# NingZhang1/pyscf_isdf

Measured on AMD Instinct MI355X. Metric: isdf_build_plus_get_jk_wall_time, lower is better.
Workload: dtype f64

## Files before the change

### include/mi355_isdf.h

```cpp
#ifndef MI355_ISDF_H
#define MI355_ISDF_H

#include <stdint.h>

#ifdef __cplusplus
extern "C" {
#endif

typedef struct isdf_ctx* isdf_handle;

#define ISDF_OK 0
#define ISDF_ERR_ARG 1
#define ISDF_ERR_HIP 2
#define ISDF_ERR_LIB 3
#define ISDF_ERR_NUM 4

int isdf_abi_version(void);

int isdf_create(int device_id, isdf_handle* out);
int isdf_destroy(isdf_handle h);
int isdf_set_stream(isdf_handle h, void* hip_stream);
const char* isdf_last_error(isdf_handle h);
int64_t isdf_workspace_bytes(isdf_handle h);
int isdf_release_workspace(isdf_handle h);
// ... 82 lines not shown
                    const int64_t* d_ip, int P, double reg_rel, double* d_theta, int64_t ldt,
                    double* d_aoP, double* reg_used);

int isdf_gather_aoP(isdf_handle h, const double* d_ao, int nao, int64_t ld, const int64_t* d_ip, int P,
                    double* d_aoP);
int isdf_gram_sq(isdf_handle h, const double* d_aoP, int P, int nao, int nh, double* d_A);
int isdf_pair_gram_rows(isdf_handle h, const double* d_aoP, int P, int nao, int nh, const double* d_ao,
                        int64_t ng, int64_t ld, double* d_B, int64_t ldb);
int isdf_block_chol(isdf_handle h, const double* d_A, int P, int nblk, const int32_t* blk_off,
                    double shift_rel, double* d_D, double* shift_used);
int isdf_block_solve(isdf_handle h, const double* d_D, int P, int nblk, const int32_t* blk_off, int side,
                     int trans, double* d_X, int64_t n, int64_t ldx);
int isdf_block_invert(isdf_handle h, const double* d_D, int P, int nblk, const int32_t* blk_off, double* d_Dinv);
int isdf_block_apply(isdf_handle h, const double* d_Dinv, int64_t ldd, int nblk, const int32_t* blk_off,
                     double* d_X, int64_t n, int64_t ldx);
int isdf_pair_rows_block_apply(isdf_handle h, const double* d_aoP, int P, int nao, const double* d_ao, int64_t ng,
                               int64_t ld, const double* d_Dinv, int64_t ldd, int nblk, const int32_t* blk_off,
                               double* d_B, int64_t ldb);
int isdf_pair_rows_squared(isdf_handle h, const double* d_aoP, int rows, int nao, const double* d_ao, int64_t ng,
                           int64_t ld, int* squared);
int isdf_pair_rows_frontier(isdf_handle h, const double* d_aoP, int nnew, int nao, const double* d_ao, int64_t ng,
                            int64_t ld, int squared, const double* d_Dinv, int64_t ldd, int nblk, const int32_t* blk_off,
                            double* d_B, int64_t ldb, int have);

int isdf_gram_prod(isdf_handle h, const double* d_aoP, int P, int nao, const double* d_psiP, int nocc, double* d_A);
int isdf_pair_prod_rows(isdf_handle h, const double* d_aoP, int P, int nao, const double* d_psiP, int nocc,
                        const double* d_ao, int64_t ld, const double* d_psi, int64_t ldpsi, int64_t ng,
                        double* d_B, int64_t ldb);
int isdf_factor_solve_half(isdf_handle h, const double* d_fac, int P, int backward, double* d_X, int64_t n, int64_t ldx);
int isdf_gram_prod_cplx(isdf_handle h, const double* d_aoP, int P, int nao, int nh, const double* d_psiP, int npsi, int npsi_h,
                        double* d_A);
int isdf_pair_prod_rows_cplx(isdf_handle h, const double* d_aoP, int P, int nao, int nh, const double* d_psiP, int npsi,
                             int npsi_h, const double* d_ao, int64_t ld, const double* d_psi, int64_t ldpsi, int64_t ng,
                             double* d_B, int64_t ldb);

int isdf_shift_diag(isdf_handle h, double* d_A, int P, double shift_rel);
int isdf_chol_inplace(isdf_handle h, double* d_A, int P, double shift_rel, double* d_scratch, double* reg_used);

int isdf_factor_solve(isdf_handle h, const double* d_fac, int P, double* d_X, int64_t n, int64_t ldx);

int isdf_bj_probe_vectors(isdf_handle h, double* d_T, int n, const double* d_fac, const double* d_D, int P,
                          int nblk, const int32_t* blk_off);
int isdf_rows_combine(isdf_handle h, const double* d_E, int n, int64_t ldE, int rows, const double* d_Y,
                      int64_t ng, int64_t ldy, double* d_F, int64_t ldf, int accumulate);

int isdf_bj_probe_rows(isdf_handle h, double* d_T, int n, const double* d_fac, const double* d_D, int P, int nblk,
// ... 136 lines not shown
```

### pyscf_isdf_amd/backend.py

```python
import ctypes
import os
import numpy as np
import torch
from . import lib as _lib

_vp = ctypes.c_void_p


def _np_ptr(a):
    return a.ctypes.data_as(_vp)


class HipBackend:
    name = 'hip-gfx950'

    def __init__(self, device=0):
        if not torch.cuda.is_available():
            raise _lib.IsdfError('no GPU visible to torch; the ISDF path has no CPU fallback')
        self.device = torch.device('cuda', device)
        torch.cuda.set_device(self.device)
        self.handle = _lib.Handle(device)
        if os.environ.get('ISDF_TRSM') == 'subst':
            self.set_option('trsm_substitution', 1)
        if os.environ.get('ISDF_OWN_FFT') in ('0', '1', '2'):
# ... 286 lines not shown
        self._stream()
        blk_off = np.ascontiguousarray(blk_off, dtype=np.int32)
        assert aoP.stride(1) == 1 and aoP.stride(0) == aoP.shape[1]
        self.handle.call('isdf_pair_rows_block_apply', self._p(aoP), aoP.shape[0], aoP.shape[1], self._p(ao), int(ng), ao.stride(0),
                         self._p(Dinv), Dinv.stride(0), len(blk_off) - 1, _np_ptr(blk_off), self._p(B), B.stride(0))

    def pair_rows_squared(self, aoP, rows, ao, ng):
        self._stream()
        sq = ctypes.c_int(0)
        self.handle.call('isdf_pair_rows_squared', self._p(aoP), int(rows), aoP.shape[1], self._p(ao), int(ng), ao.stride(0),
                         ctypes.byref(sq))
        return bool(sq.value)

    def pair_rows_frontier(self, aoP_new, ao, ng, squared, Dinv, blk_off, B, have):
        self._stream()
        blk_off = np.ascontiguousarray(blk_off, dtype=np.int32)
        nnew = aoP_new.shape[0]
        assert aoP_new.stride(1) == 1 and aoP_new.stride(0) == aoP_new.shape[1] and B.stride(1) == 1
        assert have + nnew <= B.shape[0] and blk_off[0] == 0 and blk_off[-1] <= have + nnew and B.shape[1] >= ng
        assert len(blk_off) == 1 or (Dinv.shape[0] >= blk_off[-1] and Dinv.shape[1] >= blk_off[-1])
        self.handle.call('isdf_pair_rows_frontier', self._p(aoP_new) if nnew else None, nnew, aoP_new.shape[1], self._p(ao), int(ng),
                         ao.stride(0), int(bool(squared)), self._p(Dinv) if len(blk_off) > 1 else None, Dinv.stride(0) if len(blk_off) > 1 else 0,
                         len(blk_off) - 1, _np_ptr(blk_off), self._p(B), B.stride(0), int(have))

    def shift_diag(self, A, shift_rel):
        self._stream()
        self.handle.call('isdf_shift_diag', self._p(A), A.shape[0], float(shift_rel))

    def chol_inplace(self, A, shift_rel, scratch=None):
        self._stream()
        reg = ctypes.c_double(0.0)
        assert scratch is None or scratch.numel() >= A.numel()
        self.handle.call('isdf_chol_inplace', self._p(A), A.shape[0], float(shift_rel),
                         self._p(scratch) if scratch is not None else None, ctypes.byref(reg))
        return reg.value

    def factor_solve(self, fac, X):
        self._stream()
        self.handle.call('isdf_factor_solve', self._p(fac), fac.shape[0], self._p(X), X.shape[1], X.stride(0))

    def bj_probe_rows(self, T, fac, D, blk_off, Yp, ng, F):
        self._stream()
        blk_off = np.ascontiguousarray(blk_off, dtype=np.int32)
        self.handle.call('isdf_bj_probe_rows', self._p(T), T.shape[0], self._p(fac), self._p(D), D.shape[0],
                         len(blk_off) - 1, _np_ptr(blk_off), self._p(Yp), int(ng), Yp.stride(0), self._p(F), F.stride(0))

# ... 448 lines not shown
```

### pyscf_isdf_amd/csrc/common.h

```cpp
#pragma once
#include <hip/hip_runtime.h>
#include <rocblas/rocblas.h>
#include <rocsolver/rocsolver.h>
#include <hipfft/hipfft.h>
#include <cstdint>
#include <cstdio>
#include <cstring>
#include <string>
#include <vector>
#include <map>
#include "../../include/mi355_isdf.h"

struct FftPlan {
  hipfftHandle fwd = 0, bwd = 0;
  size_t work_bytes = 0;
};

struct ProfRec {
  hipEvent_t e0 = nullptr, e1 = nullptr;
};
struct ProfEntry {
  std::vector<ProfRec> recs;
  double work = 0.0;
  double ms = 0.0;
// ... 9 lines not shown
};

struct isdf_ctx {
  int profiling = 0;
  std::map<std::string, ProfEntry> prof;
  int device = 0;
  hipStream_t stream = nullptr;
  rocblas_handle blas = nullptr;
  std::string err;
  std::map<std::vector<int>, FftPlan> plans;
  std::map<std::string, std::pair<void*, size_t>> ws;
  int num_cu = 256;
  int trsm_substitution = 0;
  int own_fft = 2;
  int gemm_nn_own = 0;
  int attr_gemm_b = 0, attr_gemm_nn = 0, attr_gemm_nn_had = 0, attr_gram_tri = 0, attr_herm = 0;
  int cand_gram = 1;
  int conv_pipe = 1;
  int conv_sub_rows = 0;
  int gram_pivot_tpb = 256;
  int gram_compact = 1;
  int gram_compact_permille = 875;
  int block_apply_waves = 16;
  int block_apply_reg = 1;
  double coul_omega = 0.0;
  double coul_rc = 0.0;
  int coul_sphere = 0;
  WsKernel wsk;
};

int isdf_fail(isdf_handle h, int code, const char* fmt, ...);
void* isdf_ws(isdf_handle h, const char* name, size_t bytes);
int isdf_get_plan(isdf_handle h, const int32_t mesh[3], int batch, FftPlan** out);
int get_coulG_half(isdf_handle h, const int32_t mesh[3], const double a[9], double extra_scale, double** out);
bool conv_rows_own_supported(const int32_t mesh[3], int nb);
bool conv_rows_q_own_supported(isdf_handle h, const int32_t mesh[3], int nb);
bool spectral_rows_own_supported(isdf_handle h, const int32_t mesh[3], int nb);
int spectral_rows_own(isdf_handle h, const double* d_in, int nb, const int32_t mesh[3], const int32_t* d_idx, const double* d_scale,
                      int npts, double* d_out, int64_t ldx, HIP_vector_type<double, 2u>* zbuf);
int spectral_lines_tile(const int32_t mesh[3]);
int spectral_rows_lines_own(isdf_handle h, const double* d_in, int nb, const int32_t mesh[3], int npts, const int32_t* d_lines,
                            int nlines_pad, const int32_t* d_slot, const double* d_slot_scale, double* d_out, int64_t ldx,
                            HIP_vector_type<double, 2u>* zbuf);
int conv_rows_q_own(isdf_handle h, const double* d_in, double* d_re, double* d_im, int nb, const int32_t mesh[3], const double* tab,
                    double2* zhalf, double2* zfull);
int conv_rows_own(isdf_handle h, const double* d_in, double* d_out, int nb, const int32_t mesh[3], const double* cg,
// ... 37 lines not shown
    if (!h || !h->profiling) return;
    ent = &h->prof[name];
    ent->work += work;
    ent->launches += launches;
    if (hipEventCreate(&rec.e0) != hipSuccess || hipEventCreate(&rec.e1) != hipSuccess) { ent = nullptr; return; }
    (void)hipEventRecord(rec.e0, h->stream);
  }
  ~ProfScope() {
    if (!ent) return;
    (void)hipEventRecord(rec.e1, h->stream);
    ent->recs.push_back(rec);
  }
};

int gemm_nt_f64(isdf_handle h, int M, int N, int64_t K, double alpha, const double* A, int64_t lda,
                const double* B, int64_t ldb, double beta, double* C, int64_t ldc);
int gemm_nt_f64_scaled(isdf_handle h, int M, int N, int64_t K, double alpha, const double* A, int64_t lda,
                       const double* B, int64_t ldb, const double* kscale, double beta, double* C,
                       int64_t ldc);
int trsm_lower_left(isdf_handle h, bool trans, int m, int64_t n, const double* L, int64_t ldl, double* X, int64_t ldx);
int trsm_lower_right(isdf_handle h, bool trans, int m, int64_t n, const double* L, int64_t ldl, double* X, int64_t ldx);
int block_forward_solve(isdf_handle h, const double* D, int64_t ldd, int nblk, const int32_t* blk_off_host, double* X,
                        int64_t ldx, int64_t n, bool own_columns = false);
int block_apply_inverse(isdf_handle h, const double* Dinv, int64_t ldd, int nblk, const int32_t* blk_off_host, double* X,
                        int64_t ldx, int64_t n, bool square_input = false);
int transpose_rm(isdf_handle h, const double* src, int64_t lds, int64_t rows, int64_t cols, double* dst, int64_t ldd);
int tri_left(isdf_handle h, bool trans, int m, int64_t n, const double* L, int64_t ldl, double* X, int64_t ldx);
int tri_right(isdf_handle h, bool trans, int m, int64_t n, const double* L, int64_t ldl, double* X, int64_t ldx);
bool gemm_nn_f64_supported(isdf_handle h, int64_t M, int64_t N, int64_t K, const double* A, int64_t lda, const double* B,
                           int64_t ldb);
int gemm_nn_f64(isdf_handle h, int64_t M, int64_t N, int64_t K, const double* A, int64_t lda, const double* B, int64_t ldb,
                double* C, int64_t ldc, bool square);
int gemm_rm(isdf_handle h, char opA, char opB, int64_t M, int64_t N, int64_t K, double alpha,
            const double* A, int64_t lda, const double* B, int64_t ldb, double beta, double* C,
            int64_t ldc);

__host__ __device__ inline int64_t gram_tri_row(int64_t r) {
  const int64_t tm = r >> 8;
  return 32768 * tm * (tm + 1) + (r & 255) * ((tm + 1) << 8);
}
static inline int64_t gram_tri_size(int64_t m) { return m > 0 ? gram_tri_row(m - 1) + (((m - 1) >> 8) + 1) * 256 : 0; }
struct GramTriUnit { int blk, tm, tn, pad; };
int gram_tri_blocks(isdf_handle h, const double* X, int64_t ldx, int K, const GramTriUnit* d_units, int64_t nunits,
                    const int64_t* d_blk_off, int64_t row0, const int64_t* d_tri_off, double* S, double flop);
```

### pyscf_isdf_amd/csrc/fit.hip

```cpp
#include "common.h"
#include <cstdlib>

namespace {

__global__ void gather_T_kernel(const double* __restrict__ L, int64_t ldL,
                                const int64_t* __restrict__ piv, int k, double* __restrict__ T) {
  const int s = blockIdx.x * blockDim.x + threadIdx.x;
  const int t = blockIdx.y;
  if (s >= k) return;
  T[(int64_t)t * k + s] = (s >= t) ? L[(int64_t)t * ldL + piv[s]] : 0.0;
}

__global__ void square_kernel(double* __restrict__ x, int64_t rows, int64_t cols, int64_t ld) {
  const int64_t c = (int64_t)blockIdx.x * blockDim.x + threadIdx.x;
  const int64_t r = blockIdx.y;
  if (c >= cols) return;
  const double v = x[r * ld + c];
  x[r * ld + c] = v * v;
}

__global__ void square_add_kernel(double* __restrict__ x, int64_t ld, const double* __restrict__ y, int64_t ldy,
                                  int64_t cols) {
  const int64_t c = (int64_t)blockIdx.x * blockDim.x + threadIdx.x;
  const int64_t r = blockIdx.y;
// ... 381 lines not shown
  return block_apply_inverse(h, d_Dinv, ldd, nblk, blk_off, d_X, ldx, n);
}

extern "C" int isdf_pair_rows_block_apply(isdf_handle h, const double* d_aoP, int P, int nao, const double* d_ao, int64_t ng,
                                          int64_t ld, const double* d_Dinv, int64_t ldd, int nblk, const int32_t* blk_off,
                                          double* d_B, int64_t ldb) {
  if (!h) return ISDF_ERR_ARG;
  ARG_CHECK(h, d_aoP && d_ao && d_Dinv && d_B && blk_off && P > 0 && nao > 0 && ng > 0 && ld >= ng && ldb >= ng && nblk > 0);
  ARG_CHECK(h, blk_off[0] == 0 && blk_off[nblk] == P);
  const bool own = gemm_nn_f64_supported(h, P, ng, nao, d_aoP, nao, d_ao, ld);
  int rc = product_rows(h, P, ng, nao, d_aoP, d_ao, ld, d_B, ldb, own);
  if (rc) return rc;
  return block_apply_inverse(h, d_Dinv, ldd, nblk, blk_off, d_B, ldb, ng, !own);
}

extern "C" int isdf_pair_rows_squared(isdf_handle h, const double* d_aoP, int rows, int nao, const double* d_ao, int64_t ng,
                                      int64_t ld, int* squared) {
  if (!h) return ISDF_ERR_ARG;
  ARG_CHECK(h, d_aoP && d_ao && squared && rows > 0 && nao > 0 && ng > 0 && ld >= ng);
  *squared = gemm_nn_f64_supported(h, rows, ng, nao, d_aoP, nao, d_ao, ld) ? 1 : 0;
  return ISDF_OK;
}

extern "C" int isdf_pair_rows_frontier(isdf_handle h, const double* d_aoP, int nnew, int nao, const double* d_ao, int64_t ng,
                                       int64_t ld, int squared, const double* d_Dinv, int64_t ldd, int nblk,
                                       const int32_t* blk_off, double* d_B, int64_t ldb, int have) {
  if (!h) return ISDF_ERR_ARG;
  ARG_CHECK(h, d_ao && d_B && nnew >= 0 && nnew <= 65535 && have >= 0 && nblk >= 0 && nao > 0 && ng > 0 && ld >= ng && ldb >= ng);
  ARG_CHECK(h, (nnew == 0 || d_aoP) && (nblk == 0 || (d_Dinv && blk_off && blk_off[0] == 0 && blk_off[nblk] <= have + nnew)));
  if (nnew > 0) {
    double* rows = d_B + (int64_t)have * ldb;
    int rc = squared ? product_rows(h, nnew, ng, nao, d_aoP, d_ao, ld, rows, ldb, true)
                     : gemm_rm(h, 'N', 'N', nnew, ng, nao, 1.0, d_aoP, nao, d_ao, ld, 0.0, rows, ldb);
    if (rc) return rc;
  }
  if (nblk == 0) return ISDF_OK;
  return block_apply_inverse(h, d_Dinv, ldd, nblk, blk_off, d_B, ldb, ng, !squared);
}

extern "C" int isdf_shift_diag(isdf_handle h, double* d_A, int P, double shift_rel) {
  if (!h) return ISDF_ERR_ARG;
  ARG_CHECK(h, d_A && P > 0 && shift_rel >= 0);
  if (shift_rel == 0.0) return ISDF_OK;
  int* info = (int*)isdf_ws(h, "fit_info", 256);
  if (!info) return ISDF_ERR_HIP;
  double* maxdiag = (double*)(info + 16);
  hipLaunchKernelGGL(max_diag_kernel, dim3(1), dim3(256), 0, h->stream, d_A, P, maxdiag);
  hipLaunchKernelGGL(add_diag_kernel, dim3((unsigned)cdiv(P, 256)), dim3(256), 0, h->stream, d_A, P, maxdiag, shift_rel);
  KERNEL_CHECK(h);
  return ISDF_OK;
}

extern "C" int isdf_chol_inplace(isdf_handle h, double* d_A, int P, double shift_rel, double* d_scratch,
                                 double* reg_used) {
  if (!h) return ISDF_ERR_ARG;
  ARG_CHECK(h, d_A && P > 0 && shift_rel >= 0);
  int* info = (int*)isdf_ws(h, "fit_info", 256);
  double* keep = d_scratch ? d_scratch : (double*)isdf_ws(h, "chol_keep", sizeof(double) * (size_t)P * P);
  if (!info || !keep) return ISDF_ERR_HIP;
  double* maxdiag = (double*)(info + 16);
// ... 243 lines not shown
```

### pyscf_isdf_amd/csrc/handle.hip

```cpp
#include "common.h"
#include <cstdarg>

int isdf_fail(isdf_handle h, int code, const char* fmt, ...) {
  char buf[1024];
  va_list ap;
  va_start(ap, fmt);
  vsnprintf(buf, sizeof(buf), fmt, ap);
  va_end(ap);
  if (h) h->err = buf;
  else fprintf(stderr, "mi355_isdf: %s\n", buf);
  return code;
}

void* isdf_ws(isdf_handle h, const char* name, size_t bytes) {
  auto& slot = h->ws[name];
  if (slot.second >= bytes && slot.first) return slot.first;
  if (slot.first) {
    (void)hipStreamSynchronize(h->stream);
    (void)hipFree(slot.first);
    slot.first = nullptr;
    slot.second = 0;
  }
  void* p = nullptr;
  hipError_t e = hipMalloc(&p, bytes ? bytes : 8);
// ... 65 lines not shown

int isdf_set_option(isdf_handle h, const char* key, int value) {
  if (!h) return ISDF_ERR_ARG;
  ARG_CHECK(h, key != nullptr);
  if (std::string(key) == "trsm_substitution") { h->trsm_substitution = value ? 1 : 0; return ISDF_OK; }
  if (std::string(key) == "own_fft") { h->own_fft = value < 0 ? 0 : (value > 2 ? 2 : value); return ISDF_OK; }
  if (std::string(key) == "gemm_nn_own") { h->gemm_nn_own = value ? 1 : 0; return ISDF_OK; }
  if (std::string(key) == "coul_sphere") { h->coul_sphere = value < 0 ? 0 : value; return ISDF_OK; }
  if (std::string(key) == "conv_pipe") { h->conv_pipe = value != 0; return ISDF_OK; }
  if (std::string(key) == "conv_sub_rows") { h->conv_sub_rows = value < 0 ? 0 : value; return ISDF_OK; }
  if (std::string(key) == "gram_pivot_tpb") {
    if (value != 64 && value != 128 && value != 256) return ISDF_ERR_ARG;
    h->gram_pivot_tpb = value;
    return ISDF_OK;
  }
  if (std::string(key) == "cand_gram") { h->cand_gram = value ? 1 : 0; return ISDF_OK; }
  if (std::string(key) == "gram_compact") { h->gram_compact = value ? 1 : 0; return ISDF_OK; }
  if (std::string(key) == "gram_compact_permille") {
    if (value < 1 || value > 1000) return isdf_fail(h, ISDF_ERR_ARG, "isdf_set_option: gram_compact_permille %d not in [1, 1000]", value);
    h->gram_compact_permille = value;
    return ISDF_OK;
  }
  if (std::string(key) == "block_apply_waves") { h->block_apply_waves = value < 1 ? 1 : value; return ISDF_OK; }
  if (std::string(key) == "block_apply_reg") { h->block_apply_reg = value ? 1 : 0; return ISDF_OK; }
  return isdf_fail(h, ISDF_ERR_ARG, "isdf_set_option: unknown key '%s'", key);
}

int isdf_create(int device_id, isdf_handle* out) {
  if (!out) return ISDF_ERR_ARG;
  *out = nullptr;
  int ndev = 0;
  hipError_t e = hipGetDeviceCount(&ndev);
  if (e != hipSuccess || ndev == 0)
    return isdf_fail(nullptr, ISDF_ERR_HIP, "no HIP device visible (%s)", hipGetErrorString(e));
  if (device_id < 0 || device_id >= ndev)
    return isdf_fail(nullptr, ISDF_ERR_ARG, "device %d out of range (%d devices)", device_id, ndev);
  isdf_ctx* h = new isdf_ctx();
  h->device = device_id;
  if (hipSetDevice(device_id) != hipSuccess) { delete h; return ISDF_ERR_HIP; }
  hipDeviceProp_t prop;
  if (hipGetDeviceProperties(&prop, device_id) == hipSuccess) h->num_cu = prop.multiProcessorCount;
  if (rocblas_create_handle(&h->blas) != rocblas_status_success) {
    delete h;
    return isdf_fail(nullptr, ISDF_ERR_LIB, "rocblas_create_handle failed");
  }
  rocblas_set_pointer_mode(h->blas, rocblas_pointer_mode_host);
// ... 84 lines not shown
```

### pyscf_isdf_amd/csrc/trsm.hip

```cpp
#include "common.h"
#include <cstdlib>

namespace {

constexpr int SB = 64;

template <bool TRANS>
__global__ __launch_bounds__(256) void subst_kernel(const double* __restrict__ L, int64_t ldl, int nb,
                                                    double* __restrict__ X, int64_t ldx, int64_t n) {
  const int64_t c = (int64_t)blockIdx.x * 256 + threadIdx.x;
  if (c >= n) return;
  double x[SB];
#pragma unroll
  for (int i = 0; i < SB; ++i) x[i] = (i < nb) ? X[(int64_t)i * ldx + c] : 0.0;
  if (!TRANS) {
#pragma unroll
    for (int i = 0; i < SB; ++i) {
      if (i < nb) {
        double s = x[i];
#pragma unroll
        for (int k = 0; k < i; ++k) s = fma(-L[(int64_t)i * ldl + k], x[k], s);
        x[i] = s / L[(int64_t)i * ldl + i];
      }
    }
// ... 125 lines not shown
    for (int k0 = 0; k0 < kend; k0 += 32) {
      if (k0 + 32 < kend) {
#pragma unroll
        for (int j = 0; j < 8; ++j) a_nxt[j] = (rowok && k0 + 32 + 8 * fk + j < m) ? pa[k0 + 32 + j] : 0.0;
      }
#pragma unroll
      for (int j = 0; j < 8; ++j)
#pragma unroll
        for (int ct = 0; ct < TN / 16; ++ct)
          acc[ct] = __builtin_amdgcn_mfma_f64_16x16x4f64(a_cur[j], pb[(k0 + j) * LDB + ct * 16], acc[ct], 0, 0, 0);
#pragma unroll
      for (int j = 0; j < 8; ++j) a_cur[j] = a_nxt[j];
    }
#pragma unroll
    for (int ct = 0; ct < TN / 16; ++ct)
#pragma unroll
      for (int r = 0; r < 4; ++r) {
        const int row = rt * 16 + fk + 4 * r, col = ct * 16 + fr;
        if (row < m && col < ncol) Xb[(int64_t)row * ldx + col] = acc[ct][r];
      }
  }
}

template <int NT, int NCT, bool SQ>
__global__ __launch_bounds__(64 * ((NT + 1) / 2)) __attribute__((amdgpu_waves_per_eu(1, 2))) void block_apply_reg_kernel(const double* __restrict__ Dinv, int64_t ldd,
                                                                            const int32_t* __restrict__ blk_off,
                                                                            double* __restrict__ X, int64_t ldx, int64_t n) {
  constexpr int TN = 16 * NCT;
  constexpr int LDB = TN + 2;
  constexpr int NPAIR = (NT + 1) / 2;
  constexpr int NTHREADS = 64 * NPAIR;
  constexpr int NCH = NT / 2 + 1;
  constexpr int MP = 16 * NT;
  constexpr int NPRE = (MP * TN + NTHREADS - 1) / NTHREADS;
  extern __shared__ double sB[];
  const int b = blockIdx.y;
  const int off = blk_off[b], m = blk_off[b + 1] - off;
  if (m <= 0) return;
  const int pair = threadIdx.x >> 6, lane = threadIdx.x & 63;
  const int fr = lane & 15, fk = lane >> 4;
  const int tA = pair, tB = NT - 1 - pair;
  const int nchA = (tA + 2) / 2, nchB = (tB == tA) ? 0 : (tB + 2) / 2;
  double a[8 * NCH];
#pragma unroll
  for (int c = 0; c < NCH; ++c) {
    const bool isA = c < nchA;
    const int t = isA ? tA : tB;
    const int k0 = 32 * (isA ? c : c - nchA) + 8 * fk;
    const int row = t * 16 + fr;
    const bool live = (c < nchA + nchB) && row < m;
    const double* pa = Dinv + (int64_t)(off + (live ? row : 0)) * ldd + off + k0;
#pragma unroll
    for (int j = 0; j < 8; ++j) a[8 * c + j] = (live && k0 + j < m) ? pa[j] : 0.0;
  }
  const int64_t ntile = (n + TN - 1) / TN;
  double pre[NPRE];
  const int r0 = threadIdx.x / TN, cc = threadIdx.x % TN;
  constexpr int RSTEP = NTHREADS / TN;
  double* const Xrow = X + (int64_t)(off + r0) * ldx + cc;
  auto fetch = [&](int64_t tile) {
    const int64_t c0 = tile * TN;
    const bool colok = c0 + cc < n;
#pragma unroll
    for (int i = 0; i < NPRE; ++i) {
      const int r = r0 + i * RSTEP;
      pre[i] = (r < m && colok) ? Xrow[(int64_t)i * RSTEP * ldx + c0] : 0.0;
    }
  };
  int64_t tile = blockIdx.x;
  if (tile < ntile) fetch(tile);
  for (; tile < ntile; tile += gridDim.x) {
#pragma unroll
    for (int i = 0; i < NPRE; ++i) {
      const int r = r0 + i * RSTEP;
      if (r < MP) {
        const double v = pre[i];
        sB[r * LDB + cc] = SQ ? v * v : v;
// ... 12 lines not shown
          const double* q = pb + (32 * c) * LDB;
#pragma unroll
          for (int j = 0; j < 8; ++j) accA = __builtin_amdgcn_mfma_f64_16x16x4f64(a[8 * c + j], q[j * LDB], accA, 0, 0, 0);
        } else if (c < nchA + nchB) {
          const double* q = pb + (32 * (c - nchA)) * LDB;
#pragma unroll
          for (int j = 0; j < 8; ++j) accB = __builtin_amdgcn_mfma_f64_16x16x4f64(a[8 * c + j], q[j * LDB], accB, 0, 0, 0);
        }
        __builtin_amdgcn_sched_barrier(0);
      }
      const int64_t col = c0 + ct * 16 + fr;
      if (col < n) {
        double* Xb = X + (int64_t)off * ldx + col;
#pragma unroll
        for (int r = 0; r < 4; ++r) {
          const int rowA = tA * 16 + fk + 4 * r;
          if (rowA < m) Xb[(int64_t)rowA * ldx] = accA[r];
          if (nchB > 0) {
            const int rowB = tB * 16 + fk + 4 * r;
            if (rowB < m) Xb[(int64_t)rowB * ldx] = accB[r];
          }
        }
      }
    }
    __syncthreads();
  }
}

template <int NT, int NCT>
static int block_apply_reg_launch(isdf_handle h, const double* Dinv, int64_t ldd, int nblk, const int32_t* d_off, double* X,
                                  int64_t ldx, int64_t n, bool sq) {
  constexpr int TN = 16 * NCT;
  constexpr int NTHREADS = 64 * ((NT + 1) / 2);
  static_assert(NTHREADS % TN == 0 && (16 * NT * TN) % NTHREADS == 0, "tile elements must divide evenly over the threads");
  const size_t lds = (size_t)16 * NT * (TN + 2) * sizeof(double);
  const int64_t ntile = (n + TN - 1) / TN;
  const unsigned gx = (unsigned)std::max<int64_t>(1, std::min<int64_t>(ntile, ((int64_t)h->num_cu * h->block_apply_waves + nblk - 1) / nblk));
  if (sq) {
    if (lds > 64 * 1024)
      HIP_TRY(h, hipFuncSetAttribute((const void*)&block_apply_reg_kernel<NT, NCT, true>, hipFuncAttributeMaxDynamicSharedMemorySize, 160 * 1024));
    hipLaunchKernelGGL(HIP_KERNEL_NAME(block_apply_reg_kernel<NT, NCT, true>), dim3(gx, (unsigned)nblk), dim3(NTHREADS), lds, h->stream,
                       Dinv, ldd, d_off, X, ldx, n);
  } else {
    if (lds > 64 * 1024)
      HIP_TRY(h, hipFuncSetAttribute((const void*)&block_apply_reg_kernel<NT, NCT, false>, hipFuncAttributeMaxDynamicSharedMemorySize, 160 * 1024));
    hipLaunchKernelGGL(HIP_KERNEL_NAME(block_apply_reg_kernel<NT, NCT, false>), dim3(gx, (unsigned)nblk), dim3(NTHREADS), lds, h->stream,
                       Dinv, ldd, d_off, X, ldx, n);
  }
  KERNEL_CHECK(h);
  return ISDF_OK;
}

template <int TN, bool SQ>
static hipError_t block_apply_lds_attr() {
  return hipFuncSetAttribute((const void*)&block_apply_mfma_kernel<TN, SQ>, hipFuncAttributeMaxDynamicSharedMemorySize, 160 * 1024);
}

int block_apply_inverse(isdf_handle h, const double* Dinv, int64_t ldd, int nblk, const int32_t* blk_off_host, double* X,
                        int64_t ldx, int64_t n, bool square_input) {
  ARG_CHECK(h, Dinv && X && blk_off_host && nblk > 0 && n > 0 && nblk <= 65535);
  int mmax = 0;
  for (int b = 0; b < nblk; ++b) mmax = std::max(mmax, blk_off_host[b + 1] - blk_off_host[b]);
  const int mpad = (mmax + 31) & ~31;
  ARG_CHECK(h, mmax > 0);
  const bool reg = h->block_apply_reg && mmax <= 256;
  const int nt = (mmax + 15) / 16;
  int tn = 0;
  const char* label;
  if (reg) {
    label = nt <= 8 ? "block_apply_reg_kernel<8,2>[byte]" : nt <= 10 ? "block_apply_reg_kernel<10,2>[byte]"
          : nt <= 12 ? "block_apply_reg_kernel<12,2>[byte]" : "block_apply_reg_kernel<16,1>[byte]";
  } else if ((size_t)mpad * (64 + 2) * sizeof(double) <= 52 * 1024) {
    tn = 64; label = "block_apply_mfma_kernel<64>[byte]";
  } else if ((size_t)mpad * (32 + 2) * sizeof(double) <= 80 * 1024) {
    tn = 32; label = "block_apply_mfma_kernel<32>[byte]";
  } else {
    ARG_CHECK(h, (size_t)mpad * (16 + 2) * sizeof(double) <= 160 * 1024);
    tn = 16; label = "block_apply_mfma_kernel<16>[byte]";
  }
  int32_t* d_off = (int32_t*)isdf_ws(h, "trsm_blk_off", sizeof(int32_t) * (size_t)(nblk + 1));
  if (!d_off) return ISDF_ERR_HIP;
  HIP_TRY(h, hipMemcpyAsync(d_off, blk_off_host, sizeof(int32_t) * (size_t)(nblk + 1), hipMemcpyHostToDevice, h->stream));
  ProfScope ps(h, label, 16.0 * (double)blk_off_host[nblk] * (double)n);
  if (reg) {
    if (nt <= 8) return block_apply_reg_launch<8, 2>(h, Dinv, ldd, nblk, d_off, X, ldx, n, square_input);
    if (nt <= 10) return block_apply_reg_launch<10, 2>(h, Dinv, ldd, nblk, d_off, X, ldx, n, square_input);
    if (nt <= 12) return block_apply_reg_launch<12, 2>(h, Dinv, ldd, nblk, d_off, X, ldx, n, square_input);
    return block_apply_reg_launch<16, 1>(h, Dinv, ldd, nblk, d_off, X, ldx, n, square_input);
  }
#define ISDF_BA_LAUNCH(TN_, SQ_)                                                                                       \
  do {                                                                                                                 \
    if ((size_t)mpad * (TN_ + 2) * sizeof(double) > 64 * 1024) {                                                       \
      HIP_TRY(h, (block_apply_lds_attr<TN_, SQ_>()));                                                                  \
    }                                                                                                                  \
    hipLaunchKernelGGL(HIP_KERNEL_NAME(block_apply_mfma_kernel<TN_, SQ_>), dim3((unsigned)cdiv(n, TN_), (unsigned)nblk),   \
                       dim3(256), (size_t)mpad * (TN_ + 2) * sizeof(double), h->stream, Dinv, ldd, d_off, X, ldx, n);  \
  } while (0)
  if (tn == 64) {
    if (square_input) ISDF_BA_LAUNCH(64, true); else ISDF_BA_LAUNCH(64, false);
  } else if (tn == 32) {
    if (square_input) ISDF_BA_LAUNCH(32, true); else ISDF_BA_LAUNCH(32, false);
  } else {
    if (square_input) ISDF_BA_LAUNCH(16, true); else ISDF_BA_LAUNCH(16, false);
  }
#undef ISDF_BA_LAUNCH
// ... 177 lines not shown
```

### pyscf_isdf_amd/fit_route.py

```python
import numpy as np


def spectral_line_plan(idx, scale, mesh, tile):
    idx = np.asarray(idx, dtype=np.int64)
    n0, n1, n2 = (int(x) for x in mesh)
    per = n1 * (n2 // 2 + 1)
    line, kx = idx % per, idx // per
    real = np.unique(line)
    lines = np.full(-(-len(real) // 16) * 16, -1, dtype=np.int32)
    lines[:len(real)] = real
    slot = np.full((len(lines), n0), -1, dtype=np.int32)
    where = np.searchsorted(real, line)
    slot[where, kx] = np.arange(len(idx), dtype=np.int32)
    if np.count_nonzero(slot >= 0) != len(idx):
        return None
    slot = np.ascontiguousarray(slot.reshape(-1, tile, n0).transpose(0, 2, 1))
    slot_scale = np.where(slot >= 0, np.asarray(scale, dtype=np.float64)[np.maximum(slot, 0)], 0.0)
    return lines, slot, slot_scale, len(real)


class FitRouteMixin:
    def _bj_prepare(self, ao, nh, d_ip, ip_off, aoP, scratch=None):
        be = self.backend
        P = aoP.shape[0]
# ... 317 lines not shown
        P = W.shape[0]
        for b0 in range(0, P, nbat):
            b1 = min(P, b0 + nbat)
            be.gemm_nt(X[b0:b1], X[b0:], W[b0:b1, b0:], alpha=1.0)
        be.symmetrize_upper(W)
        self._bj_finish(st['Afac'], st['Dblk'], st['ip_off'], W)

    def _pair_rows_piece(self, big):
        align = int(getattr(self, 'pair_rows_align', 0) or 0)
        if align <= 0 or not hasattr(self.backend, 'pair_rows_frontier') or getattr(self, '_psi', None) is not None \
                or not self.block_apply_mfma or big > 1100:
            return 0
        return int(self.fft_batch or 512) // align * align

    def _spectral_rows_two_frontiers(self, X, scratch, piece, plan, probe):
        be, st = self.backend, self._fit_state
        ip_off = np.asarray(st['ip_off'], dtype=np.int64)
        P = int(ip_off[-1])
        mesh = np.asarray(self.mesh, dtype=np.int32)
        G = self.ao.shape[1]
        Dinv = self._block_inverse(st['Dblk'], ip_off)
        nbat = int(self.fft_batch or 512)
        squared = be.pair_rows_squared(self.aoP, min(piece, P), self.ao, G)
        app, prod = 0, 0
        while app < P:
            new = min(piece, P - prod)
            j = int(np.searchsorted(ip_off, prod + new, side='right')) - 1
            i = int(np.searchsorted(ip_off, app))
            end = int(ip_off[j])
            be.pair_rows_frontier(self.aoP[prod:prod + new], self.ao, G, squared, Dinv[app:, app:],
                                  (ip_off[i:j + 1] - app).astype(np.int32), scratch, prod - app)
            prod += new
            if end > app:
                rows = scratch[:end - app]
                if probe is not None:
                    be.rows_combine(probe[0][:, app:end], rows, probe[1], accumulate=app > 0)
                be.spectral_rows(rows, mesh, plan['idx'], plan['scale'], X[app:end], batch=min(nbat, end - app), **plan['lines_kw'])
                tail = prod - end
                if tail > 0:
                    src = scratch[end - app:prod - app]
                    scratch[:tail].copy_(src.clone() if tail > end - app else src)
                app = end

    def _bj_finish(self, Afac, Dblk, ip_off, W, antisymmetric=False):
        be = self.backend
        be.W_from_factor(Afac, 2, W)
        be.W_from_factor(Afac, 0, W)
        be.block_solve(Dblk, ip_off, 0, 1, W)
        be.block_solve(Dblk, ip_off, 1, 0, W)
        be.symmetrize_mean(W, antisymmetric)

    def _bj_clusters(self):
        cell = self.cell
        natm = cell.natm
        parent = list(range(natm))

        def find(i):
            while parent[i] != i:
# ... 117 lines not shown
```

### pyscf_isdf_amd/lib.py

```python
import ctypes
import os

_HERE = os.path.dirname(os.path.abspath(__file__))
LIB_PATH = os.path.join(_HERE, 'lib', 'libmi355_isdf.so')
ABI_VERSION = 21

_lib = None

c_int, c_i64, c_dbl, c_vp = ctypes.c_int, ctypes.c_int64, ctypes.c_double, ctypes.c_void_p

SIGNATURES = {
    'isdf_abi_version': (c_int, []),
    'isdf_create': (c_int, [c_int, ctypes.POINTER(c_vp)]),
    'isdf_destroy': (c_int, [c_vp]),
    'isdf_set_stream': (c_int, [c_vp, c_vp]),
    'isdf_last_error': (ctypes.c_char_p, [c_vp]),
    'isdf_workspace_bytes': (c_i64, [c_vp]),
    'isdf_set_coulomb_omega': (c_int, [c_vp, c_dbl]),
    'isdf_set_coulomb_cutoff': (c_int, [c_vp, c_dbl]),
    'isdf_set_coulomb_ws': (c_int, [c_vp, c_dbl, c_vp, c_vp, c_vp, c_vp]),
    'isdf_set_option': (c_int, [c_vp, ctypes.c_char_p, c_int]),
    'isdf_release_workspace': (c_int, [c_vp]),
    'isdf_prof_enable': (c_int, [c_vp, c_int]),
    'isdf_prof_reset': (c_int, [c_vp]),
# ... 8 lines not shown
                                  c_i64]),
    'isdf_select_ip_work_bytes': (c_i64, [c_int, c_i64]),
    'isdf_select_ip_gram': (c_int, [c_vp, c_vp, c_int, c_i64, c_int, c_dbl, c_dbl, c_int, c_vp, ctypes.POINTER(ctypes.c_int32)]),
    'isdf_fit_from_chol': (c_int, [c_vp, c_vp, c_int, c_i64, c_i64, c_vp]),
    'isdf_fit_prepare': (c_int, [c_vp, c_vp, c_int, c_i64, c_vp, c_int, c_dbl, c_vp, c_vp, ctypes.POINTER(c_dbl)]),
    'isdf_fit_apply': (c_int, [c_vp, c_vp, c_vp, c_int, c_int, c_vp, c_i64, c_i64, c_int, c_vp, c_i64]),
    'isdf_gather_aoP': (c_int, [c_vp, c_vp, c_int, c_i64, c_vp, c_int, c_vp]),
    'isdf_gram_sq': (c_int, [c_vp, c_vp, c_int, c_int, c_int, c_vp]),
    'isdf_pair_gram_rows': (c_int, [c_vp, c_vp, c_int, c_int, c_int, c_vp, c_i64, c_i64, c_vp, c_i64]),
    'isdf_gram_prod': (c_int, [c_vp, c_vp, c_int, c_int, c_vp, c_int, c_vp]),
    'isdf_pair_prod_rows': (c_int, [c_vp, c_vp, c_int, c_int, c_vp, c_int, c_vp, c_i64, c_vp, c_i64, c_i64, c_vp, c_i64]),
    'isdf_factor_solve_half': (c_int, [c_vp, c_vp, c_int, c_int, c_vp, c_i64, c_i64]),
    'isdf_gram_prod_cplx': (c_int, [c_vp, c_vp, c_int, c_int, c_int, c_vp, c_int, c_int, c_vp]),
    'isdf_pair_prod_rows_cplx': (c_int, [c_vp, c_vp, c_int, c_int, c_int, c_vp, c_int, c_int, c_vp, c_i64, c_vp, c_i64, c_i64,
                                         c_vp, c_i64]),
    'isdf_block_chol': (c_int, [c_vp, c_vp, c_int, c_int, c_vp, c_dbl, c_vp, ctypes.POINTER(c_dbl)]),
    'isdf_block_solve': (c_int, [c_vp, c_vp, c_int, c_int, c_vp, c_int, c_int, c_vp, c_i64, c_i64]),
    'isdf_block_invert': (c_int, [c_vp, c_vp, c_int, c_int, c_vp, c_vp]),
    'isdf_block_apply': (c_int, [c_vp, c_vp, c_i64, c_int, c_vp, c_vp, c_i64, c_i64]),
    'isdf_pair_rows_block_apply': (c_int, [c_vp, c_vp, c_int, c_int, c_vp, c_i64, c_i64, c_vp, c_i64, c_int, c_vp, c_vp, c_i64]),
    'isdf_pair_rows_squared': (c_int, [c_vp, c_vp, c_int, c_int, c_vp, c_i64, c_i64, ctypes.POINTER(c_int)]),
    'isdf_pair_rows_frontier': (c_int, [c_vp, c_vp, c_int, c_int, c_vp, c_i64, c_i64, c_int, c_vp, c_i64, c_int, c_vp, c_vp, c_i64,
                                        c_int]),
    'isdf_shift_diag': (c_int, [c_vp, c_vp, c_int, c_dbl]),
    'isdf_chol_inplace': (c_int, [c_vp, c_vp, c_int, c_dbl, c_vp, ctypes.POINTER(c_dbl)]),
    'isdf_factor_solve': (c_int, [c_vp, c_vp, c_int, c_vp, c_i64, c_i64]),
    'isdf_bj_probe_vectors': (c_int, [c_vp, c_vp, c_int, c_vp, c_vp, c_int, c_int, c_vp]),
    'isdf_rows_combine': (c_int, [c_vp, c_vp, c_int, c_i64, c_int, c_vp, c_i64, c_i64, c_vp, c_i64, c_int]),
    'isdf_bj_probe_rows': (c_int, [c_vp, c_vp, c_int, c_vp, c_vp, c_int, c_int, c_vp, c_vp, c_i64, c_i64, c_vp, c_i64]),
    'isdf_gather_T': (c_int, [c_vp, c_vp, c_int, c_i64, c_vp, c_vp]),
    'isdf_W_from_factor': (c_int, [c_vp, c_vp, c_int, c_int, c_vp, c_i64]),
    'isdf_fit_global': (c_int, [c_vp, c_vp, c_int, c_i64, c_i64, c_vp, c_int, c_dbl, c_vp, c_i64, c_vp, ctypes.POINTER(c_dbl)]),
    'isdf_coulomb_W': (c_int, [c_vp, c_vp, c_int, c_i64, c_vp, c_vp, c_int, c_int, c_int, c_int, c_vp, c_i64]),
    'isdf_coulomb_rows': (c_int, [c_vp, c_vp, c_int, c_i64, c_vp, c_vp, c_int, c_vp, c_i64]),
    'isdf_symmetrize_upper': (c_int, [c_vp, c_vp, c_int, c_i64]),
    'isdf_symmetrize_mean': (c_int, [c_vp, c_vp, c_int, c_i64, c_int]),
    'isdf_get_j': (c_int, [c_vp, c_vp, c_int, c_i64, c_i64, c_vp, c_vp, c_vp, c_int, c_vp]),
    'isdf_rho': (c_int, [c_vp, c_vp, c_int, c_i64, c_i64, c_vp, c_int, c_vp, c_i64]),
    'isdf_coulomb_potential': (c_int, [c_vp, c_vp, c_int, c_i64, c_vp, c_vp]),
    'isdf_vj_from_vR': (c_int, [c_vp, c_vp, c_int, c_i64, c_i64, c_vp, c_int, c_i64, c_vp]),
    'isdf_eval_ao_k': (c_int, [c_vp, c_vp, c_int, c_vp, c_int, c_vp, c_int, c_vp, c_int, c_vp, c_vp, c_int, c_vp, c_i64, c_vp, c_vp, c_i64]),
    'isdf_select_ip_cplx': (c_int, [c_vp, c_vp, c_int, c_int, c_i64, c_int, c_vp, c_vp, c_dbl, c_dbl, c_vp, c_i64, c_vp, c_vp]),
    'isdf_fit_prepare_cplx': (c_int, [c_vp, c_vp, c_int, c_int, c_i64, c_vp, c_int, c_dbl, c_vp, c_vp, ctypes.POINTER(c_dbl)]),
    'isdf_fit_apply_cplx': (c_int, [c_vp, c_vp, c_vp, c_int, c_int, c_int, c_vp, c_i64, c_i64, c_int, c_vp, c_i64]),
    'isdf_coulG_q': (c_int, [c_vp, c_vp, c_vp, c_vp, c_int, c_dbl, c_vp]),
    'isdf_coulomb_Wq': (c_int, [c_vp, c_vp, c_int, c_i64, c_vp, c_vp, c_dbl, c_int, c_int, c_int, c_int, c_vp, c_vp, c_i64]),
# ... 109 lines not shown
```

Measured before the change: 16.50.

## Fuse probe-row combine into block-apply-inverse kernel via MFMA partials

Adds a PROBE variant of the register block-apply kernel. While the solved rows are still in registers, it multiplies them by the probe vectors E using f64 MFMA and writes per-block partial sums. A separate reduce kernel sums the partials into F, with accumulation across block groups bounded by a workspace size option. The fit route calls this fused path when there are at most 8 probes, so the rows no longer have to be re-read by a separate rows_combine pass. In exchange it adds partial-sum workspace traffic, a reduce launch per group, and more LDS and registers in the kernel, which may lower occupancy.

```diff
diff --git a/include/mi355_isdf.h b/include/mi355_isdf.h
--- a/include/mi355_isdf.h
+++ b/include/mi355_isdf.h
@@ -128,6 +128,10 @@
 int isdf_pair_rows_frontier(isdf_handle h, const double* d_aoP, int nnew, int nao, const double* d_ao, int64_t ng,
                             int64_t ld, int squared, const double* d_Dinv, int64_t ldd, int nblk, const int32_t* blk_off,
                             double* d_B, int64_t ldb, int have);
+int isdf_pair_rows_frontier_probe(isdf_handle h, const double* d_aoP, int nnew, int nao, const double* d_ao, int64_t ng,
+                                  int64_t ld, int squared, const double* d_Dinv, int64_t ldd, int nblk, const int32_t* blk_off,
+                                  double* d_B, int64_t ldb, int have, const double* d_E, int n, int64_t ldE, double* d_F,
+                                  int64_t ldf, int accumulate);
 
 int isdf_gram_prod(isdf_handle h, const double* d_aoP, int P, int nao, const double* d_psiP, int nocc, double* d_A);
 int isdf_pair_prod_rows(isdf_handle h, const double* d_aoP, int P, int nao, const double* d_psiP, int nocc,
diff --git a/pyscf_isdf_amd/backend.py b/pyscf_isdf_amd/backend.py
--- a/pyscf_isdf_amd/backend.py
+++ b/pyscf_isdf_amd/backend.py
@@ -332,6 +332,19 @@
         self.handle.call('isdf_pair_rows_frontier', self._p(aoP_new) if nnew else None, nnew, aoP_new.shape[1], self._p(ao), int(ng),
                          ao.stride(0), int(bool(squared)), self._p(Dinv) if len(blk_off) > 1 else None, Dinv.stride(0) if len(blk_off) > 1 else 0,
                          len(blk_off) - 1, _np_ptr(blk_off), self._p(B), B.stride(0), int(have))
+
+    def pair_rows_frontier_probe(self, aoP_new, ao, ng, squared, Dinv, blk_off, B, have, E, F, accumulate=False):
+        self._stream()
+        blk_off = np.ascontiguousarray(blk_off, dtype=np.int32)
+        nnew = aoP_new.shape[0]
+        assert aoP_new.stride(1) == 1 and aoP_new.stride(0) == aoP_new.shape[1] and B.stride(1) == 1
+        assert have + nnew <= B.shape[0] and blk_off[0] == 0 and blk_off[-1] <= have + nnew and B.shape[1] >= ng
+        assert len(blk_off) == 1 or (Dinv.shape[0] >= blk_off[-1] and Dinv.shape[1] >= blk_off[-1])
+        assert E.stride(1) == 1 and F.stride(1) == 1 and E.shape[0] == F.shape[0] <= 8 and E.shape[1] == blk_off[-1] and F.shape[1] >= ng
+        self.handle.call('isdf_pair_rows_frontier_probe', self._p(aoP_new) if nnew else None, nnew, aoP_new.shape[1], self._p(ao),
+                         int(ng), ao.stride(0), int(bool(squared)), self._p(Dinv) if len(blk_off) > 1 else None,
+                         Dinv.stride(0) if len(blk_off) > 1 else 0, len(blk_off) - 1, _np_ptr(blk_off), self._p(B), B.stride(0),
+                         int(have), self._p(E), E.shape[0], E.stride(0), self._p(F), F.stride(0), int(bool(accumulate)))
 
     def shift_diag(self, A, shift_rel):
         self._stream()
diff --git a/pyscf_isdf_amd/csrc/common.h b/pyscf_isdf_amd/csrc/common.h
--- a/pyscf_isdf_amd/csrc/common.h
+++ b/pyscf_isdf_amd/csrc/common.h
@@ -55,6 +55,7 @@
   int gram_compact = 1;
   int gram_compact_permille = 875;
   int block_apply_waves = 16;
+  int probe_ws_mib = 512;
   int block_apply_reg = 1;
   double coul_omega = 0.0;
   double coul_rc = 0.0;
@@ -138,8 +139,9 @@
 int trsm_lower_right(isdf_handle h, bool trans, int m, int64_t n, const double* L, int64_t ldl, double* X, int64_t ldx);
 int block_forward_solve(isdf_handle h, const double* D, int64_t ldd, int nblk, const int32_t* blk_off_host, double* X,
                         int64_t ldx, int64_t n, bool own_columns = false);
+struct BlockProbe { const double* E; int64_t ldE; int n; double* F; int64_t ldf; int accumulate; };
 int block_apply_inverse(isdf_handle h, const double* Dinv, int64_t ldd, int nblk, const int32_t* blk_off_host, double* X,
-                        int64_t ldx, int64_t n, bool square_input = false);
+                        int64_t ldx, int64_t n, bool square_input = false, const BlockProbe* probe = nullptr);
 int transpose_rm(isdf_handle h, const double* src, int64_t lds, int64_t rows, int64_t cols, double* dst, int64_t ldd);
 int tri_left(isdf_handle h, bool trans, int m, int64_t n, const double* L, int64_t ldl, double* X, int64_t ldx);
 int tri_right(isdf_handle h, bool trans, int m, int64_t n, const double* L, int64_t ldl, double* X, int64_t ldx);
diff --git a/pyscf_isdf_amd/csrc/fit.hip b/pyscf_isdf_amd/csrc/fit.hip
--- a/pyscf_isdf_amd/csrc/fit.hip
+++ b/pyscf_isdf_amd/csrc/fit.hip
@@ -427,9 +427,9 @@
   return ISDF_OK;
 }
 
-extern "C" int isdf_pair_rows_frontier(isdf_handle h, const double* d_aoP, int nnew, int nao, const double* d_ao, int64_t ng,
-                                       int64_t ld, int squared, const double* d_Dinv, int64_t ldd, int nblk,
-                                       const int32_t* blk_off, double* d_B, int64_t ldb, int have) {
+static int pair_rows_frontier(isdf_handle h, const double* d_aoP, int nnew, int nao, const double* d_ao, int64_t ng,
+                              int64_t ld, int squared, const double* d_Dinv, int64_t ldd, int nblk,
+                              const int32_t* blk_off, double* d_B, int64_t ldb, int have, const BlockProbe* probe) {
   if (!h) return ISDF_ERR_ARG;
   ARG_CHECK(h, d_ao && d_B && nnew >= 0 && nnew <= 65535 && have >= 0 && nblk >= 0 && nao > 0 && ng > 0 && ld >= ng && ldb >= ng);
   ARG_CHECK(h, (nnew == 0 || d_aoP) && (nblk == 0 || (d_Dinv && blk_off && blk_off[0] == 0 && blk_off[nblk] <= have + nnew)));
@@ -440,7 +440,23 @@
     if (rc) return rc;
   }
   if (nblk == 0) return ISDF_OK;
-  return block_apply_inverse(h, d_Dinv, ldd, nblk, blk_off, d_B, ldb, ng, !squared);
+  return block_apply_inverse(h, d_Dinv, ldd, nblk, blk_off, d_B, ldb, ng, !squared, probe);
+}
+
+extern "C" int isdf_pair_rows_frontier(isdf_handle h, const double* d_aoP, int nnew, int nao, const double* d_ao, int64_t ng,
+                                       int64_t ld, int squared, const double* d_Dinv, int64_t ldd, int nblk,
+                                       const int32_t* blk_off, double* d_B, int64_t ldb, int have) {
+  return pair_rows_frontier(h, d_aoP, nnew, nao, d_ao, ng, ld, squared, d_Dinv, ldd, nblk, blk_off, d_B, ldb, have, nullptr);
+}
+
+extern "C" int isdf_pair_rows_frontier_probe(isdf_handle h, const double* d_aoP, int nnew, int nao, const double* d_ao, int64_t ng,
+                                             int64_t ld, int squared, const double* d_Dinv, int64_t ldd, int nblk,
+                                             const int32_t* blk_off, double* d_B, int64_t ldb, int have, const double* d_E, int n,
+                                             int64_t ldE, double* d_F, int64_t ldf, int accumulate) {
+  if (!h) return ISDF_ERR_ARG;
+  ARG_CHECK(h, d_E && d_F && n > 0 && n <= 8 && ldf >= ng && (nblk == 0 || (blk_off && ldE >= blk_off[nblk])));
+  const BlockProbe probe = {d_E, ldE, n, d_F, ldf, accumulate};
+  return pair_rows_frontier(h, d_aoP, nnew, nao, d_ao, ng, ld, squared, d_Dinv, ldd, nblk, blk_off, d_B, ldb, have, &probe);
 }
 
 extern "C" int isdf_shift_diag(isdf_handle h, double* d_A, int P, double shift_rel) {
diff --git a/pyscf_isdf_amd/csrc/handle.hip b/pyscf_isdf_amd/csrc/handle.hip
--- a/pyscf_isdf_amd/csrc/handle.hip
+++ b/pyscf_isdf_amd/csrc/handle.hip
@@ -111,6 +111,7 @@
     return ISDF_OK;
   }
   if (std::string(key) == "block_apply_waves") { h->block_apply_waves = value < 1 ? 1 : value; return ISDF_OK; }
+  if (std::string(key) == "probe_ws_mib") { h->probe_ws_mib = value < 1 ? 1 : value; return ISDF_OK; }
   if (std::string(key) == "block_apply_reg") { h->block_apply_reg = value ? 1 : 0; return ISDF_OK; }
   return isdf_fail(h, ISDF_ERR_ARG, "isdf_set_option: unknown key '%s'", key);
 }
diff --git a/pyscf_isdf_amd/csrc/trsm.hip b/pyscf_isdf_amd/csrc/trsm.hip
--- a/pyscf_isdf_amd/csrc/trsm.hip
+++ b/pyscf_isdf_amd/csrc/trsm.hip
@@ -171,10 +171,12 @@
   }
 }
 
-template <int NT, int NCT, bool SQ>
+template <int NT, int NCT, bool SQ, bool PROBE>
 __global__ __launch_bounds__(64 * ((NT + 1) / 2)) __attribute__((amdgpu_waves_per_eu(1, 2))) void block_apply_reg_kernel(const double* __restrict__ Dinv, int64_t ldd,
                                                                             const int32_t* __restrict__ blk_off,
-                                                                            double* __restrict__ X, int64_t ldx, int64_t n) {
+                                                                            double* __restrict__ X, int64_t ldx, int64_t n,
+                                                                            const double* __restrict__ E, int64_t ldE, int nE,
+                                                                            double* __restrict__ Fp) {
   constexpr int TN = 16 * NCT;
   constexpr int LDB = TN + 2;
   constexpr int NPAIR = (NT + 1) / 2;
@@ -202,6 +204,17 @@
 #pragma unroll
     for (int j = 0; j < 8; ++j) a[8 * c + j] = (live && k0 + j < m) ? pa[j] : 0.0;
   }
+  double eA[4], eB[4];
+  double* const sF = sB + MP * LDB;
+  if (PROBE) {
+    static_assert(!PROBE || NTHREADS >= 8 * TN, "one thread per (probe row, column) of a tile");
+#pragma unroll
+    for (int r = 0; r < 4; ++r) {
+      const int rowA = tA * 16 + fk + 4 * r, rowB = tB * 16 + fk + 4 * r;
+      eA[r] = (fr < nE && rowA < m) ? E[(int64_t)fr * ldE + off + rowA] : 0.0;
+      eB[r] = (fr < nE && nchB > 0 && rowB < m) ? E[(int64_t)fr * ldE + off + rowB] : 0.0;
+    }
+  }
   const int64_t ntile = (n + TN - 1) / TN;
   double pre[NPRE];
   const int r0 = threadIdx.x / TN, cc = threadIdx.x % TN;
@@ -260,33 +273,73 @@
           }
         }
       }
+      if (PROBE) {
+        d4v f = (d4v){0.0, 0.0, 0.0, 0.0};
+#pragma unroll
+        for (int r = 0; r < 4; ++r) f = __builtin_amdgcn_mfma_f64_16x16x4f64(eA[r], accA[r], f, 0, 0, 0);
+        if (nchB > 0) {
+#pragma unroll
+          for (int r = 0; r < 4; ++r) f = __builtin_amdgcn_mfma_f64_16x16x4f64(eB[r], accB[r], f, 0, 0, 0);
+        }
+        double* q = sF + (pair * 8 + fk) * TN + 16 * ct + fr;
+        q[0] = f[0];
+        q[4 * TN] = f[1];
+      }
     }
     __syncthreads();
-  }
+    if (PROBE && threadIdx.x < 8 * TN) {
+      const int j = threadIdx.x / TN, cl = threadIdx.x % TN;
+      if (j < nE && c0 + cl < n) {
+        double s = sF[j * TN + cl];
+#pragma unroll
+        for (int p = 1; p < NPAIR; ++p) s += sF[(p * 8 + j) * TN + cl];
+        Fp[((int64_t)b * nE + j) * n + c0 + cl] = s;
+      }
+    }
+  }
+}
+
+__global__ __launch_bounds__(256) void probe_reduce_kernel(const double* __restrict__ Fp, const int32_t* __restrict__ blk_off,
+                                                           int nblk, int nE, int64_t n, double* __restrict__ F, int64_t ldf,
+                                                           int accumulate) {
+  const int64_t g = (int64_t)blockIdx.x * 256 + threadIdx.x;
+  const int j = blockIdx.y;
+  if (g >= n) return;
+  double s = accumulate ? F[(int64_t)j * ldf + g] : 0.0;
+  for (int b = 0; b < nblk; ++b)
+    if (blk_off[b + 1] > blk_off[b]) s += Fp[((int64_t)b * nE + j) * n + g];
+  F[(int64_t)j * ldf + g] = s;
+}
+
+template <int NT, int NCT, bool SQ, bool PROBE>
+static int block_apply_reg_launch1(isdf_handle h, const double* Dinv, int64_t ldd, int nblk, const int32_t* d_off, double* X,
+                                   int64_t ldx, int64_t n, unsigned gx, const double* E, int64_t ldE, int nE, double* Fp) {
+  constexpr int TN = 16 * NCT;
+  constexpr int NPAIR = (NT + 1) / 2;
+  const size_t lds = ((size_t)16 * NT * (TN + 2) + (PROBE ? NPAIR * 8 * TN : 0)) * sizeof(double);
+  if (lds > 64 * 1024)
+    HIP_TRY(h, hipFuncSetAttribute((const void*)&block_apply_reg_kernel<NT, NCT, SQ, PROBE>, hipFuncAttributeMaxDynamicSharedMemorySize, 160 * 1024));
+  hipLaunchKernelGGL(HIP_KERNEL_NAME(block_apply_reg_kernel<NT, NCT, SQ, PROBE>), dim3(gx, (unsigned)nblk), dim3(64 * NPAIR), lds, h->stream,
+                     Dinv, ldd, d_off, X, ldx, n, E, ldE, nE, Fp);
+  KERNEL_CHECK(h);
+  return ISDF_OK;
 }
 
 template <int NT, int NCT>
 static int block_apply_reg_launch(isdf_handle h, const double* Dinv, int64_t ldd, int nblk, const int32_t* d_off, double* X,
-                                  int64_t ldx, int64_t n, bool sq) {
+                                  int64_t ldx, int64_t n, bool sq, const double* E = nullptr, int64_t ldE = 0, int nE = 0,
+                                  double* Fp = nullptr) {
   constexpr int TN = 16 * NCT;
   constexpr int NTHREADS = 64 * ((NT + 1) / 2);
   static_assert(NTHREADS % TN == 0 && (16 * NT * TN) % NTHREADS == 0, "tile elements must divide evenly over the threads");
-  const size_t lds = (size_t)16 * NT * (TN + 2) * sizeof(double);
   const int64_t ntile = (n + TN - 1) / TN;
   const unsigned gx = (unsigned)std::max<int64_t>(1, std::min<int64_t>(ntile, ((int64_t)h->num_cu * h->block_apply_waves + nblk - 1) / nblk));
-  if (sq) {
-    if (lds > 64 * 1024)
-      HIP_TRY(h, hipFuncSetAttribute((const void*)&block_apply_reg_kernel<NT, NCT, true>, hipFuncAttributeMaxDynamicSharedMemorySize, 160 * 1024));
-    hipLaunchKernelGGL(HIP_KERNEL_NAME(block_apply_reg_kernel<NT, NCT, true>), dim3(gx, (unsigned)nblk), dim3(NTHREADS), lds, h->stream,
-                       Dinv, ldd, d_off, X, ldx, n);
-  } else {
-    if (lds > 64 * 1024)
-      HIP_TRY(h, hipFuncSetAttribute((const void*)&block_apply_reg_kernel<NT, NCT, false>, hipFuncAttributeMaxDynamicSharedMemorySize, 160 * 1024));
-    hipLaunchKernelGGL(HIP_KERNEL_NAME(block_apply_reg_kernel<NT, NCT, false>), dim3(gx, (unsigned)nblk), dim3(NTHREADS), lds, h->stream,
-                       Dinv, ldd, d_off, X, ldx, n);
-  }
-  KERNEL_CHECK(h);
-  return ISDF_OK;
+  if (E) {
+    if (sq) return block_apply_reg_launch1<NT, NCT, true, true>(h, Dinv, ldd, nblk, d_off, X, ldx, n, gx, E, ldE, nE, Fp);
+    return block_apply_reg_launch1<NT, NCT, false, true>(h, Dinv, ldd, nblk, d_off, X, ldx, n, gx, E, ldE, nE, Fp);
+  }
+  if (sq) return block_apply_reg_launch1<NT, NCT, true, false>(h, Dinv, ldd, nblk, d_off, X, ldx, n, gx, nullptr, 0, 0, nullptr);
+  return block_apply_reg_launch1<NT, NCT, false, false>(h, Dinv, ldd, nblk, d_off, X, ldx, n, gx, nullptr, 0, 0, nullptr);
 }
 
 template <int TN, bool SQ>
@@ -294,8 +347,9 @@
   return hipFuncSetAttribute((const void*)&block_apply_mfma_kernel<TN, SQ>, hipFuncAttributeMaxDynamicSharedMemorySize, 160 * 1024);
 }
 
+
 int block_apply_inverse(isdf_handle h, const double* Dinv, int64_t ldd, int nblk, const int32_t* blk_off_host, double* X,
-                        int64_t ldx, int64_t n, bool square_input) {
+                        int64_t ldx, int64_t n, bool square_input, const BlockProbe* probe) {
   ARG_CHECK(h, Dinv && X && blk_off_host && nblk > 0 && n > 0 && nblk <= 65535);
   int mmax = 0;
   for (int b = 0; b < nblk; ++b) mmax = std::max(mmax, blk_off_host[b + 1] - blk_off_host[b]);
@@ -319,6 +373,32 @@
   int32_t* d_off = (int32_t*)isdf_ws(h, "trsm_blk_off", sizeof(int32_t) * (size_t)(nblk + 1));
   if (!d_off) return ISDF_ERR_HIP;
   HIP_TRY(h, hipMemcpyAsync(d_off, blk_off_host, sizeof(int32_t) * (size_t)(nblk + 1), hipMemcpyHostToDevice, h->stream));
+  if (probe) {
+    ARG_CHECK(h, probe->E && probe->F && probe->n > 0 && probe->n <= 8 && probe->ldE >= blk_off_host[nblk] && probe->ldf >= n);
+    if (!reg) {
+      int rc = block_apply_inverse(h, Dinv, ldd, nblk, blk_off_host, X, ldx, n, square_input, nullptr);
+      if (rc) return rc;
+      return isdf_rows_combine(h, probe->E, probe->n, probe->ldE, blk_off_host[nblk], X, n, ldx, probe->F, probe->ldf,
+                               probe->accumulate);
+    }
+    const int gmax = (int)std::max<size_t>(1, ((size_t)h->probe_ws_mib << 20) / (sizeof(double) * (size_t)probe->n * (size_t)n));
+    const int gsz = std::min(nblk, gmax);
+    double* Fp = (double*)isdf_ws(h, "gemm_partials", sizeof(double) * (size_t)gsz * probe->n * (size_t)n);
+    if (!Fp) return ISDF_ERR_HIP;
+    ProfScope ps(h, label, 16.0 * (double)blk_off_host[nblk] * (double)n);
+    for (int g0 = 0; g0 < nblk; g0 += gsz) {
+      const int ng_ = std::min(gsz, nblk - g0);
+      int rc = nt <= 8    ? block_apply_reg_launch<8, 2>(h, Dinv, ldd, ng_, d_off + g0, X, ldx, n, square_input, probe->E, probe->ldE, probe->n, Fp)
+               : nt <= 10 ? block_apply_reg_launch<10, 2>(h, Dinv, ldd, ng_, d_off + g0, X, ldx, n, square_input, probe->E, probe->ldE, probe->n, Fp)
+               : nt <= 12 ? block_apply_reg_launch<12, 2>(h, Dinv, ldd, ng_, d_off + g0, X, ldx, n, square_input, probe->E, probe->ldE, probe->n, Fp)
+                          : block_apply_reg_launch<16, 1>(h, Dinv, ldd, ng_, d_off + g0, X, ldx, n, square_input, probe->E, probe->ldE, probe->n, Fp);
+      if (rc) return rc;
+      hipLaunchKernelGGL(probe_reduce_kernel, dim3((unsigned)cdiv(n, 256), (unsigned)probe->n), dim3(256), 0, h->stream, Fp,
+                         d_off + g0, ng_, probe->n, n, probe->F, probe->ldf, (probe->accumulate || g0 > 0) ? 1 : 0);
+      KERNEL_CHECK(h);
+    }
+    return ISDF_OK;
+  }
   ProfScope ps(h, label, 16.0 * (double)blk_off_host[nblk] * (double)n);
   if (reg) {
     if (nt <= 8) return block_apply_reg_launch<8, 2>(h, Dinv, ldd, nblk, d_off, X, ldx, n, square_input);
diff --git a/pyscf_isdf_amd/fit_route.py b/pyscf_isdf_amd/fit_route.py
--- a/pyscf_isdf_amd/fit_route.py
+++ b/pyscf_isdf_amd/fit_route.py
@@ -363,18 +363,25 @@
         Dinv = self._block_inverse(st['Dblk'], ip_off)
         nbat = int(self.fft_batch or 512)
         squared = be.pair_rows_squared(self.aoP, min(piece, P), self.ao, G)
+        fused = probe is not None and probe[0].shape[0] <= 8 and getattr(self, 'w_probe_fused', True) \
+            and hasattr(be, 'pair_rows_frontier_probe')
         app, prod = 0, 0
         while app < P:
             new = min(piece, P - prod)
             j = int(np.searchsorted(ip_off, prod + new, side='right')) - 1
             i = int(np.searchsorted(ip_off, app))
             end = int(ip_off[j])
-            be.pair_rows_frontier(self.aoP[prod:prod + new], self.ao, G, squared, Dinv[app:, app:],
-                                  (ip_off[i:j + 1] - app).astype(np.int32), scratch, prod - app)
+            if fused and end > app:
+                be.pair_rows_frontier_probe(self.aoP[prod:prod + new], self.ao, G, squared, Dinv[app:, app:],
+                                            (ip_off[i:j + 1] - app).astype(np.int32), scratch, prod - app,
+                                            probe[0][:, app:end], probe[1], accumulate=app > 0)
+            else:
+                be.pair_rows_frontier(self.aoP[prod:prod + new], self.ao, G, squared, Dinv[app:, app:],
+                                      (ip_off[i:j + 1] - app).astype(np.int32), scratch, prod - app)
             prod += new
             if end > app:
                 rows = scratch[:end - app]
-                if probe is not None:
+                if probe is not None and not fused:
                     be.rows_combine(probe[0][:, app:end], rows, probe[1], accumulate=app > 0)
                 be.spectral_rows(rows, mesh, plan['idx'], plan['scale'], X[app:end], batch=min(nbat, end - app), **plan['lines_kw'])
                 tail = prod - end
diff --git a/pyscf_isdf_amd/lib.py b/pyscf_isdf_amd/lib.py
--- a/pyscf_isdf_amd/lib.py
+++ b/pyscf_isdf_amd/lib.py
@@ -54,6 +54,8 @@
     'isdf_pair_rows_squared': (c_int, [c_vp, c_vp, c_int, c_int, c_vp, c_i64, c_i64, ctypes.POINTER(c_int)]),
     'isdf_pair_rows_frontier': (c_int, [c_vp, c_vp, c_int, c_int, c_vp, c_i64, c_i64, c_int, c_vp, c_i64, c_int, c_vp, c_vp, c_i64,
                                         c_int]),
+    'isdf_pair_rows_frontier_probe': (c_int, [c_vp, c_vp, c_int, c_int, c_vp, c_i64, c_i64, c_int, c_vp, c_i64, c_int, c_vp, c_vp,
+                                              c_i64, c_int, c_vp, c_int, c_i64, c_vp, c_i64, c_int]),
     'isdf_shift_diag': (c_int, [c_vp, c_vp, c_int, c_dbl]),
     'isdf_chol_inplace': (c_int, [c_vp, c_vp, c_int, c_dbl, c_vp, ctypes.POINTER(c_dbl)]),
     'isdf_factor_solve': (c_int, [c_vp, c_vp, c_int, c_vp, c_i64, c_i64]),
```

New measurement: 16.45 (median of 4 runs). About the same (-0.3%).
